# CODEJIN/multi_speaker_tts

Hardware: AMD Instinct MI355X
Metric: mel-frames/sec (train step) at batch 32x(128 tok,800 mel) (higher is better)
Workload: dtype f32

## Files before the change

include/mstts.h:

```cpp
#ifndef MSTTS_H_
#define MSTTS_H_
#include <stdint.h>
#ifdef __cplusplus
extern "C" {
#endif

typedef void* mstts_stream_t;

enum { MSTTS_OK = 0, MSTTS_ERR_SHAPE = -1, MSTTS_ERR_DTYPE = -2, MSTTS_ERR_ALIGN = -3, MSTTS_ERR_LAUNCH = -4 };
enum { MSTTS_ACT_NONE = 0, MSTTS_ACT_RELU = 1, MSTTS_ACT_TANH = 2, MSTTS_ACT_SIGMOID = 3 };

const char* mstts_last_error(void);
int mstts_abi_version(void);
int mstts_debug_park_cus(int32_t n_workgroups, int64_t microseconds, uint32_t* done_count, mstts_stream_t s);

typedef struct {
    const float* A; const float* B; float* C; const float* bias;
    int64_t M, N, K;
    int64_t lda, ldb, ldc;
    int32_t trans_a, trans_b;
    int32_t win_T, win_C, win_pad;
    int32_t act, accumulate, split_k;
    int64_t batch, stride_a, stride_b, stride_c;
    float alpha;
    int32_t win_dil;
} mstts_gemm_desc;
int mstts_gemm_f32(const mstts_gemm_desc* d, mstts_stream_t s);
int mstts_gemm_tail_split(int32_t on);
int mstts_gemm_split3(int32_t on);
int mstts_gemm_split_big(int32_t on);
int mstts_gemm_big_min_workgroups(int32_t f32_split, int32_t bf16);
int mstts_gemm_deterministic(int32_t on);
int mstts_gemm_bf16(const mstts_gemm_desc* d, mstts_stream_t s);
int mstts_gemm_bf16_autocut(int32_t on);
int mstts_gemm_bf16_big(int32_t on);

int mstts_philox_keep_mask(uint8_t* out, int64_t n, uint64_t seed, uint32_t stream_id, float keep_prob, mstts_stream_t s);
int mstts_philox_keep_mask_rows(uint8_t* out, int64_t outer, int64_t B, int64_t inner, uint64_t seed, uint32_t stream_id,
                                uint64_t sample0, float keep_prob, mstts_stream_t s);

int mstts_embedding_fwd(const int32_t* token, const float* table, float* out, int64_t n, int64_t vocab, int64_t width, mstts_stream_t s);
int mstts_embedding_bwd(const int32_t* token, const float* dout, float* dtable, int64_t n, int64_t vocab, int64_t width, mstts_stream_t s);

int mstts_bn_train_fwd(const float* x, const float* gamma, const float* beta, float* moving_mean, float* moving_var,
                       float* y, float* save_mean, float* save_rstd, const uint8_t* keep_mask, float keep_prob,
                       float momentum, float eps, int64_t rows, int64_t C, float* ws, mstts_stream_t s);
int mstts_bn_infer_fwd(const float* x, const float* gamma, const float* beta, const float* moving_mean,
                       const float* moving_var, float* y, float eps, int64_t rows, int64_t C, mstts_stream_t s);
int mstts_bn_train_bwd(const float* dy, const float* x, const float* gamma, const float* save_mean, const float* save_rstd,
                       const uint8_t* keep_mask, float keep_prob, int32_t act, float* dz, float* dgamma, float* dbeta,
                       float* dbias, int64_t rows, int64_t C, float* ws, mstts_stream_t s);

#define MSTTS_BN_SEG_MAX 16
typedef struct { const float* gamma; const float* beta; float* moving_mean; float* moving_var; } mstts_bn_seg;
typedef struct { mstts_bn_seg seg[MSTTS_BN_SEG_MAX]; } mstts_bn_seg_table;
int mstts_bn_train_fwd_seg(const float* x, int64_t ld, const mstts_bn_seg_table* segs, int32_t nseg, float* y, float* save_mean,
                           float* save_rstd, float momentum, float eps, int64_t rows, int64_t C, int64_t pool_T, float* ws, mstts_stream_t s);
#define MSTTS_BANK_MAX 16
typedef struct { const float* kernel[MSTTS_BANK_MAX]; const float* bias[MSTTS_BANK_MAX]; } mstts_convbank_src;
int mstts_convbank_pack(const mstts_convbank_src* src, int32_t bank_k, int32_t k_split, int64_t cin, int64_t cout, float* w, float* bias,
                        mstts_stream_t s);

int mstts_dropout(const float* x, const uint8_t* keep_mask, float keep_prob, float* y, int64_t n, mstts_stream_t s);
int mstts_relu_dropout_bwd(const float* dy, const float* y_saved, const uint8_t* keep_mask, float keep_prob, float* dx, int64_t n, mstts_stream_t s);
int mstts_colsum(const float* x, int64_t rows, int64_t C, int64_t ld, float* out, int32_t accumulate, mstts_stream_t s);
int mstts_add(const float* a, const float* b, float* y, int64_t n, mstts_stream_t s);
int mstts_fill(float* y, float v, int64_t n, mstts_stream_t s);
int mstts_persist_status(const uint32_t* ctrl_a, int32_t done_a, const uint32_t* ctrl_b, int32_t done_b, int32_t* flag, mstts_stream_t s);
// ... 424 lines not shown
```

multi_speaker_tts_amd/csrc/gemm.hip:

```cpp
#include "gemm_tile.h"
#include <type_traits>
#include <cmath>
#include <cstdlib>

namespace mstts {

constexpr int BK = 32;
constexpr int BN = 128;

struct GemmArgs : GemmTileArgs {
    int body, tail_s, tail_kps;
    int band;
};

template <int R, bool VEC>
struct LoaderKC {
    static constexpr int NV = R * BK / 4 / 256;
    float4 reg[NV];
    const float* ubase;
    unsigned voff[NV], rmask;
    int t_row[NV], tap, kc, ld_;
    __device__ __forceinline__ void prepare(const float* __restrict__ base, long ld, int row0, int k0, int rows,
                                            int wT, int wC, int wpad, int wdil) {
        const int k4 = threadIdx.x & 7, r = threadIdx.x >> 3;
// ... 224 lines not shown
}

template <int BM>
struct GemmF32 {
    using Args = GemmArgs;
    static constexpr int THREADS = 256;
    static constexpr size_t LDS_BYTES = 0;
    template <bool TA, bool TB, bool VEC, bool WIN> static constexpr auto kernel() { return &gemm_kernel<BM, TA, TB, VEC>; }
};

#include "gemm_split.inc"

}

using namespace mstts;

static int g_tail_split = 1;
extern "C" int mstts_gemm_tail_split(int32_t on) { g_tail_split = on != 0; return MSTTS_OK; }
static int g_split3 = 1;
extern "C" int mstts_gemm_split3(int32_t on) { g_split3 = on != 0; return MSTTS_OK; }
static int g_split_big = 1;
extern "C" int mstts_gemm_split_big(int32_t on) { g_split_big = on != 0; return MSTTS_OK; }
static int g_split_big_min = 160;
namespace mstts { void gemm_bf16_set_big_min(int n); }
extern "C" int mstts_gemm_big_min_workgroups(int32_t f32_split, int32_t bf16) {
    if (f32_split > 0) g_split_big_min = f32_split;
    gemm_bf16_set_big_min(bf16);
    return MSTTS_OK;
}
static thread_local int t_deterministic = 0;
extern "C" int mstts_gemm_deterministic(int32_t on) { t_deterministic = on != 0; return MSTTS_OK; }
namespace mstts { int gemm_deterministic_now() { return t_deterministic; } }

extern "C" int mstts_gemm_f32(const mstts_gemm_desc* d, mstts_stream_t stream) {
    GemmArgs g;
    bool vec;
    const int rc = gemm_args_from(d, "gemm", BK, 1 << 24, &g, &vec);
    if (rc != MSTTS_OK || g.M == 0 || g.N == 0) return rc;
    const int batch = d->batch > 0 ? (int)d->batch : 1, split = g.split_k, kps = g.k_per_split;
    const bool skinny = d->M <= 32;
    int bm = skinny ? 32 : 128, tail_s = 1, tail_rem = 0;
    const bool split3 = g_split3 && !skinny && d->K >= 160 && (d->win_T <= 0 || (d->win_T >= BK && d->win_C >= BK)) && gemm_ready<GemmSplit>();
    if (!skinny) {
        const double t128 = (double)cdiv(d->M, 128) * cdiv(d->N, BN) * batch * split, t64 = (double)cdiv(d->M, 64) * cdiv(d->N, BN) * batch * split;
        const double e128 = t128 / (ceil(t128 / 256.0) * 256.0), e64 = t64 / (ceil(t64 / 256.0) * 256.0);
        if (e64 * 0.95 > e128 && !split3) bm = 64;
        if (g_tail_split && !t_deterministic && batch == 1 && split == 1 && (d->act == MSTTS_ACT_NONE || !d->accumulate)) {
            double best = (bm == 128 ? ceil(t128 / 256.0) : ceil(t64 / 256.0) * 0.54);
            const int ktiles = cdiv(d->K, BK);
            for (int cand = 128; cand >= (split3 ? 128 : 64); cand -= 64) {
                const long t = (long)cdiv(d->M, cand) * cdiv(d->N, BN);
                int rem = (int)(t % 256);
                if (d->act != MSTTS_ACT_NONE) rem = (int)(t - (t - rem) / cdiv(d->N, BN) * cdiv(d->N, BN));
                if (split3 && t <= 128) rem = (int)t;
                else if (t <= 256 || rem == 0 || rem > 128) continue;
                int s = 256 / rem;
                if (s > 16) s = 16;
                if (s > ktiles / 8) s = ktiles / 8;
                if (s < 2) continue;
                const double c = ((double)(t / 256) + 1.25 / s + 0.06) * (cand == 128 ? 1.0 : 0.54);
                if (c < best) { best = c; bm = cand; tail_s = s; tail_rem = rem; }
            }
        }
    }
    hipStream_t st = (hipStream_t)stream;
    const bool ta = d->trans_a != 0, tb = d->trans_b != 0, win = g.win_T > 0;
    {
        const long big_wgs = (long)cdiv(d->M, GSB_BM) * cdiv(d->N, GSB_BN) * batch * split;
        if (split3 && g_split_big && d->M >= 192 && d->N >= 192 && big_wgs >= g_split_big_min && d->lda < (1 << 22) && d->ldb < (1 << 22) &&
            (d->win_T <= 0 || (d->win_T >= GSB_BK && d->win_C >= GSB_BK)) && (d->act == MSTTS_ACT_NONE || split == 1) && gemm_ready<GemmSplitBig>()) {
            const int kpsb = gemm_k_per_split(g.K, split, GSB_BK);
            g.k_per_split = kpsb;
            g.body = 0; g.tail_s = 1; g.tail_kps = kpsb; g.band = 0;
            dim3 gridb(cdiv(d->M, GSB_BM) * cdiv(d->N, GSB_BN), 1, batch * split);
            gemm_launch<GemmSplitBig>(g, ta, tb, vec, win, gridb, st);
            MSTTS_CHECK_LAUNCH("gemm_f32 (split, 256 x 256 tile)");
            return MSTTS_OK;
        }
    }
    const int tiles = cdiv(d->M, bm) * cdiv(d->N, BN);
    g.body = tiles; g.tail_s = 1; g.tail_kps = kps;
    g.band = (split3 && tail_s == 1 && cdiv(d->N, BN) > 8) ? 8 : 0;
    if (tail_s > 1) {
        const int rem = tail_rem, tiles_n = cdiv(d->N, BN);
        g.body = tiles - rem; g.tail_s = tail_s;
        g.tail_kps = (cdiv(g.K, BK) + tail_s - 1) / tail_s * BK;
        if (!d->accumulate) {
            const long r0 = (long)(g.body / tiles_n) * bm;
            if (hipMemset2DAsync(d->C + r0 * d->ldc, (size_t)d->ldc * 4, 0, (size_t)d->N * 4, (size_t)(d->M - r0), st) != hipSuccess)
                MSTTS_REQUIRE(false, MSTTS_ERR_LAUNCH, "gemm: clearing the tail tiles failed");
        }
    }
    dim3 grid(g.body + (tiles - g.body) * g.tail_s, 1, batch * split);
    if (split3) gemm_launch<GemmSplit>(g, ta, tb, vec, win, grid, st);
    else if (skinny) gemm_launch<GemmF32<32>>(g, ta, tb, vec, win, grid, st);
    else if (bm == 64) gemm_launch<GemmF32<64>>(g, ta, tb, vec, win, grid, st);
    else gemm_launch<GemmF32<128>>(g, ta, tb, vec, win, grid, st);
    MSTTS_CHECK_LAUNCH("gemm_f32");
    if (tail_s > 1 && d->act != MSTTS_ACT_NONE) {
        const long r0 = (long)(g.body / cdiv(d->N, BN)) * bm;
        const long n = (d->M - r0) * d->N;
        hipLaunchKernelGGL(gemm_tail_act_kernel, dim3((unsigned)cdiv(n, 256)), dim3(256), 0, st, d->C + r0 * d->ldc, d->ldc, (int)d->N, n, d->act);
        MSTTS_CHECK_LAUNCH("gemm_f32 tail activation");
    }
    return MSTTS_OK;
}
```

multi_speaker_tts_amd/csrc/gemm_split.inc:

```

typedef __bf16 gs_bf16x8 __attribute__((ext_vector_type(8)));
typedef __bf16 gs_bf16x4 __attribute__((ext_vector_type(4)));
constexpr int GS_BM = 128, GS_LD = 40;
constexpr int GS_PLANE = 128 * GS_LD;

struct Split3 { gs_bf16x4 hi, mid, lo; };
__device__ __forceinline__ uint32_t gs_cvt_pk(float a, float b) {
    uint32_t r;
    asm("v_cvt_pk_bf16_f32 %0, %1, %2" : "=v"(r) : "v"(a), "v"(b));
    return r;
}
__device__ __forceinline__ float gs_sub(float a, uint32_t b_bits) {
    float r;
    asm("v_sub_f32 %0, %1, %2" : "=v"(r) : "v"(a), "v"(b_bits));
    return r;
}
__device__ __forceinline__ void gs_split2(float x0, float x1, uint32_t& hi, uint32_t& mid, uint32_t& lo) {
    hi = gs_cvt_pk(x0, x1);
    x0 = gs_sub(x0, hi << 16); x1 = gs_sub(x1, hi & 0xffff0000u);
    mid = gs_cvt_pk(x0, x1);
    x0 = gs_sub(x0, mid << 16); x1 = gs_sub(x1, mid & 0xffff0000u);
    lo = gs_cvt_pk(x0, x1);
}
__device__ __forceinline__ Split3 gs_split4(float a, float b, float c, float d) {
// ... 123 lines not shown
    auto products = [&](int set) {
#pragma unroll
        for (int tt = 0; tt < GS_NPROD; ++tt) {
            const int pa = (tt == 0) ? 0 : (tt == 1) ? 1 : (tt == 2) ? 0 : (tt == 3) ? 1 : (tt == 4) ? 2 : 0;
            const int pb = (tt == 0) ? 0 : (tt == 1) ? 0 : (tt == 2) ? 1 : (tt == 3) ? 1 : (tt == 4) ? 0 : 2;
#pragma unroll
            for (int i = 0; i < 2; ++i)
#pragma unroll
                for (int j = 0; j < 2; ++j)
                    acc[i][j] = __builtin_amdgcn_mfma_f32_32x32x16_bf16(fa[set][i][pa], fb[set][j][pb], acc[i][j], 0, 0, 0);
        }
    };
    GS_BAR(0);
    frags(0, gs_lds, 0);
    for (int t = 0; t < nt2; ++t) {
        const __bf16* buf = gs_lds + (t & 1) * GS_BUF;
        frags(1, buf, 1);
        __builtin_amdgcn_sched_barrier(0);
        products(0);
        __builtin_amdgcn_sched_barrier(0);
        GS_BAR(0);
        frags(0, gs_lds + ((t + 1) & 1) * GS_BUF, 0);
        __builtin_amdgcn_sched_barrier(0);
        products(1);
        __builtin_amdgcn_sched_barrier(0);
    }
#ifdef GS_STAMP
    if (stamp && (threadIdx.x & 63) == 0) { unsigned long long* o = (unsigned long long*)g.bias; o[0] = acc_wait; o[1] = __builtin_readcyclecounter() - t_begin; o[2] = nt2; o[3] = wall_clock64() - w_begin; }
    if (stamp) return;
#endif
    gemm_store_tile<2, 2>(g, acc, C, m0 + wrow, n0 + wcol, lane, split == 0 && piece <= 0, g.split_k > 1 || piece >= 0);
}

constexpr int GSB_BM = 256, GSB_BN = 256, GSB_BK = 16, GSB_LD = 24, GSB_THREADS = 512;
constexpr int GSB_PLANE = 256 * GSB_LD;
constexpr int GSB_BUF = 6 * GSB_PLANE;
constexpr size_t GSB_LDS_BYTES = 2 * GSB_BUF * sizeof(__bf16);
template <bool VEC, bool WIN> using GsbLoaderKC = TileLoaderKC<4, 2, 128, GSB_LD, SplitPlanes<GSB_PLANE>, VEC, WIN>;
template <bool VEC, bool WIN> using GsbLoaderMC = TileLoaderMC<4, GSB_LD, SplitPlanes<GSB_PLANE>, VEC, WIN>;

template <bool TRANSPOSED, int HALF>
__device__ __forceinline__ bool gsb_stages(int tid) {
    if (TRANSPOSED) return (tid >> 8) == HALF;
    return true;
}

template <bool TA, bool TB, bool VEC, bool WIN>
__global__ __launch_bounds__(GSB_THREADS) void gemm_split_big_kernel(GemmArgs g) {
    extern __shared__ __attribute__((aligned(16))) __bf16 gs_lds[];
    const int tiles_n = (g.N + GSB_BN - 1) / GSB_BN;
    const int tile = gemm_xcd_tile(blockIdx.x, gridDim.x);
    const int tile_m = tile / tiles_n, tile_n = tile % tiles_n;
    const int batch = blockIdx.z / g.split_k, split = blockIdx.z % g.split_k;
    float* C = g.C + (long)batch * g.stride_c;
    const int m0 = tile_m * GSB_BM, n0 = tile_n * GSB_BN;
    const int kbeg = split * g.k_per_split;
    const int kend = min(g.K, kbeg + g.k_per_split);
    const int nt = kend > kbeg ? (kend - kbeg + GSB_BK - 1) / GSB_BK : 0;
    const int tid = threadIdx.x, lane = tid & 63, wave = __builtin_amdgcn_readfirstlane(tid >> 6);
    const int wrow = (wave >> 2) * 128, wcol = (wave & 3) * 64;
    const int l31 = lane & 31, kg = lane >> 5;

    using LA = typename std::conditional<TA, GsbLoaderMC<VEC, WIN>, GsbLoaderKC<VEC, WIN>>::type;
    using LB = typename std::conditional<TB, GsbLoaderKC<VEC, false>, GsbLoaderMC<VEC, false>>::type;
    LA la; LB lb;
    const bool a_mine = gsb_stages<TA, 0>(tid), b_mine = gsb_stages<!TB, 1>(tid);
    const int tid_a = TA ? (tid & 255) : tid, tid_b = TB ? tid : (tid & 255);
    if (a_mine) la.prepare(tid_a, g.A + (long)batch * g.stride_a, g.lda, m0, kbeg, g.M, g.win_T, g.win_C, g.win_pad, g.win_dil);
    if (b_mine) lb.prepare(tid_b, g.B + (long)batch * g.stride_b, g.ldb, n0, kbeg, g.N, 0, 1, 0, 1);
    float4 ra[4], rb[4];
    auto load = [&](int k) {
        if (a_mine) la.load(tid_a, ra, k, kend, g.lda, g.win_T, g.win_C, g.win_pad, g.win_dil);
        if (b_mine) lb.load(tid_b, rb, k, kend, g.ldb, 0, 1, 0, 1);
    };
    auto store = [&](int buf) {
        if (a_mine) la.store(tid_a, ra, gs_lds + buf * GSB_BUF);
        if (b_mine) lb.store(tid_b, rb, gs_lds + buf * GSB_BUF + 3 * GSB_PLANE);
    };

    f32x16 acc[4][2];
#pragma unroll
    for (int i = 0; i < 4; ++i)
#pragma unroll
        for (int j = 0; j < 2; ++j)
#pragma unroll
            for (int r = 0; r < 16; ++r) acc[i][j][r] = 0.f;

    const int aoff = (wrow + l31) * GSB_LD + kg * 8, boff = 3 * GSB_PLANE + (wcol + l31) * GSB_LD + kg * 8;
    gs_bf16x8 fb[2][3], fa0[4], fa1[4];
    auto ldA = [&](gs_bf16x8 (&f)[4], const __bf16* buf, int p) {
#pragma unroll
        for (int i = 0; i < 4; ++i) f[i] = *reinterpret_cast<const gs_bf16x8*>(buf + aoff + p * GSB_PLANE + i * 32 * GSB_LD);
    };
    auto ldB = [&](const __bf16* buf) {
#pragma unroll
        for (int p = 0; p < 3; ++p)
#pragma unroll
            for (int j = 0; j < 2; ++j) fb[j][p] = *reinterpret_cast<const gs_bf16x8*>(buf + boff + p * GSB_PLANE + j * 32 * GSB_LD);
    };
    auto mm = [&](const gs_bf16x8 (&f)[4], int pb) {
#pragma unroll
        for (int i = 0; i < 4; ++i)
#pragma unroll
            for (int j = 0; j < 2; ++j)
                acc[i][j] = __builtin_amdgcn_mfma_f32_32x32x16_bf16(f[i], fb[j][pb], acc[i][j], 0, 0, 0);
    };

    if (nt > 0) {
        load(kbeg);
        store(0);
        load(kbeg + GSB_BK);
        gemm_barrier();
        for (int t = 0; t < nt; ++t) {
            const __bf16* buf = gs_lds + (t & 1) * GSB_BUF;
            ldB(buf); ldA(fa0, buf, 0); ldA(fa1, buf, 1);
            mm(fa0, 0); mm(fa0, 1); mm(fa0, 2);
            ldA(fa0, buf, 2);
            store((t + 1) & 1);
            load(kbeg + (t + 2) * GSB_BK);
            mm(fa1, 0); mm(fa1, 1);
            mm(fa0, 0);
            gemm_barrier();
        }
    }
    gemm_store_tile<4, 2>(g, acc, C, m0 + wrow, n0 + wcol, lane, split == 0, g.split_k > 1);
}

struct GemmSplit {
    using Args = GemmArgs;
    static constexpr int THREADS = GS_THREADS;
    static constexpr size_t LDS_BYTES = GS_LDS_BYTES;
    template <bool TA, bool TB, bool VEC, bool WIN> static constexpr auto kernel() { return &gemm_split_kernel<TA, TB, VEC, WIN>; }
};
struct GemmSplitBig {
    using Args = GemmArgs;
    static constexpr int THREADS = GSB_THREADS;
    static constexpr size_t LDS_BYTES = GSB_LDS_BYTES;
    template <bool TA, bool TB, bool VEC, bool WIN> static constexpr auto kernel() { return &gemm_split_big_kernel<TA, TB, VEC, WIN>; }
};
```

multi_speaker_tts_amd/engine.py:

```python
from __future__ import annotations

import ctypes as C
import os
import warnings

import numpy as np
import torch

from . import lib
from .lib import ACT_NONE, ACT_RELU, ACT_TANH, gemm, ptr, call
from .masks import MaskSet, step_seed
from .params import CELL, ENC_CELL, LSA, LSA_VARS, VOC, Dims, ParamStore, bank_groups, bank_suffix
from .persist import PERSIST_COOLDOWN, PERSIST_STRIKES, CoolDown, Ticket, decoder_workgroups, lstm_bwd_workgroups, lstm_fwd_workgroups, near_xcd
from .training import (BN_EPS, BN_MOM, Engine, _split_k, _split_k_big, bn_train_fwd, conv_bn_bwd, conv_fwd, exponential_decay, lstm_layer_grads,
                       lstm_seq_bwd, lstm_seq_fwd)

MAX_PLANS = 64



def learning_rate(step):
    from . import Hyper_Parameters as hp
    return exponential_decay(hp.Train.Learning_Rate, step)


VOC_OVERLAP = os.environ.get("MSTTS_VOC_OVERLAP", "1") != "0"
VOC_FUSED = os.environ.get("MSTTS_VOC_FUSED", "1") != "0"
POSTNET_WGRAD_OVERLAP = os.environ.get("MSTTS_POSTNET_WGRAD_OVERLAP", "1") != "0"
ENC_TAIL_OVERLAP = os.environ.get("MSTTS_ENC_TAIL_OVERLAP", "1") != "0"
ENC_OVERLAP = os.environ.get("MSTTS_ENC_OVERLAP", "1") != "0"


class _WS:
    """Attribute bag of device buffers for one (B, T_enc, L) shape: views into the engine's workspace arena."""


class _LateScalars:

    def __init__(self, event, slot, wr_rate):
        self.event, self.slot, self.wr_rate, self._res = event, slot, wr_rate, None

    def get(self):
        if self._res is None:
            self.event.synchronize()
            s = self.slot.numpy().copy()
            wr = float(s[3]) * self.wr_rate
            self._res = {"Linear_Loss": float(s[0]), "Postnet_Loss": float(s[1]), "Stop_Loss": float(s[2]),
                         "Weight_Regularization_Loss": wr, "Loss": float(s[0] + s[1] + s[2]) + wr}
        return self._res


class _Arena:

    ALIGN = 256

    def __init__(self, device):
        self.device, self.buf, self.cap, self.generation = device, None, 0, 0

    def ensure(self, nbytes):
        if nbytes <= self.cap:
            return False
        self.buf = None
# ... 87 lines not shown
        self.persist_bwd_selftest = 0
        self.persist_stamps = None
        self.persist_bwd = self.persist and os.environ.get("MSTTS_PERSIST_BWD", "1") != "0" and bool(lb.mstts_persist_bwd_supported(1, H, M, d.att, 1, d.att_k))
        self.persist_bwd_fallbacks = 0
        self.ctx_dead = d.spk if d.spk == 256 and M == 2 * d.enc_lstm + d.spk else 0
        self.speaker_ticket_redos = 0
        self.trace_events, self.bptt_end_event = False, None
        self.collective_redos = 0
        self.persist_bwd_stamps = None
        if self.persist:
            self.pk = [self._f(int(lb.mstts_persist_pack_floats(i))) for i in range(3)]
        self.persist_enc = os.environ.get("MSTTS_PERSIST_ENC", "1") != "0" and bool(lb.mstts_persist_lstm_supported(1, He))
        self.persist_enc_fallbacks = 0
        if self.persist_enc:
            n = int(lb.mstts_persist_lstm_pack_floats())
            self.enc_pk = {dr: (self._f(n), self._f(n)) for dr in ("fw", "bw")}
        if self.device.type == "cuda":
            self._side = torch.cuda.Stream(device=self.device)
            self._enc_stream = torch.cuda.Stream(device=self.device)
            self._voc_stream = self._enc_stream
        if self.persist_bwd:
            self.pkb = [self._f(int(lb.mstts_persist_bwd_pack_floats(i))) for i in range(3)]
        self.flip = {}
        self.voc_bank = None
        if update_vocoder_bn and d.bank_ch % 4 == 0 and d.n_mel % 4 == 0 and 1 <= d.bank_k <= lib.BANK_MAX:
            groups = bank_groups(d.bank_k, max(1, d.bank_k // 2))
            n = sum(win * d.n_mel * (hi - lo + 1) * d.bank_ch for lo, hi, win, _ in groups)
            self.voc_bank = {"groups": groups, "w": self._f(n), "bias": self._f(d.bank_k * d.bank_ch), "version": None, "tables": None}
        self.big_tiles = os.environ.get("MSTTS_SPLIT_K_BIG", "1") != "0"
        self._derived_stale = True
        self.gemm_dtype = (gemm_dtype or "f32").lower()
        if self.gemm_dtype not in ("f32", "bf16"):
            raise ValueError("gemm_dtype must be 'f32' or 'bf16'")
        self.recurrent_dtype = (recurrent_dtype or "f32").lower()
        if self.recurrent_dtype not in ("f32", "bf16"):
            raise ValueError("recurrent_dtype must be 'f32' or 'bf16'")
        self.bf = None
        if self.recurrent_dtype == "bf16" and lb.mstts_cell_fwd_bf16_supported(H, M + H) and lb.mstts_cell_fwd_bf16_supported(H, 2 * H):
            self.w0p16 = torch.zeros((M + H) * 4 * H, dtype=torch.int16, device=self.device)
            self.w1p16 = torch.zeros(2 * H * 4 * H, dtype=torch.int16, device=self.device)
        if self.recurrent_dtype == "bf16":
            sp = (C.c_int32 * 6)()
            if not lib.load().mstts_decoder_bf16_splits(H, M, d.att, sp):
                raise ValueError("bf16 recurrent products need dec_lstm, mem and att widths that are multiples of 64")
            i16 = lambda n: torch.zeros(n, dtype=torch.int16, device=self.device)
            self.bf = {"splits": list(sp), "w0f_f": i16((M + H) * 4 * H), "w1_f": i16(2 * H * 4 * H), "wq_f": i16(H * d.att),
                       "w0f_b": i16((M + H) * 4 * H), "w1_b": i16(2 * H * 4 * H), "wq_b": i16(H * d.att)}

    def _gemm(self, *a, exact=False, **k):
        bf = self.gemm_dtype == "bf16" and not exact
        if self.deterministic and k.get("split_k", 1) > 1:
            k["split_k"], k["accumulate"] = 1, True
        if k.get("split_k", 1) > 1 and self.big_tiles:
            big = _split_k_big(a[3], a[4], a[5], None)
            if big is not None:
                k["split_k"] = max(2, big)
            elif bf:
                k["split_k"], k["accumulate"] = 1, True
        return gemm(*a, bf16=bf, **k)

    def _ensure_fallback_packs(self):
        if not getattr(self, "_fallback_packs_stale", True):
            return
        self._fallback_packs_stale = False
        d = self.d
        H, M = d.dec_lstm, d.mem
# ... 168 lines not shown
        w.mel_out = f(B, S, d.n_mel)
        w.bn_ws = f(2 * max(d.post_ch, d.enc_conv_ch, d.bank_k * d.bank_ch, d.proj1_ch, d.n_mel, d.emb))
        if self.update_vocoder_bn:
            w.voc_fused = VOC_FUSED and self.voc_bank is not None
            if not w.voc_fused:
                w.v_tmp = f(B * S, d.bank_ch)
                w.v_tmp2 = f(B * S, d.bank_ch)
                w.v_p2y = f(B * S, d.n_mel)
            w.v_cat = f(B * S, d.bank_k * d.bank_ch)
            w.v_pool = f(B * S, d.bank_k * d.bank_ch)
            w.v_p1 = f(B * S, d.proj1_ch)
            w.v_p1y = f(B * S, d.proj1_ch)
            w.v_p2 = f(B * S, d.n_mel)
            widest = max(d.bank_k * d.bank_ch if w.voc_fused else d.bank_ch, d.proj1_ch, d.n_mel)
            w.v_stat = f(2 * widest)
            w.v_bn_ws = f(4 * widest)
        w.scalars = f(4)
        w.d_linear, w.d_post, w.d_stop = f(B, S, d.n_mel), f(B, S, d.n_mel), f(B, S)
        w.post_dz = [f(B * S, c) for c in chans]
        w.post_dx = f(B * S, max(d.post_ch, d.n_mel))
        w.post_dx2 = f(B * S, max(d.post_ch, d.n_mel))
        w.d_proj = f(S, B, self.proj_ld)
        w.d_pj = f(S, B, H + M, zero=bool(self.ctx_dead))
        w.dg0, w.dg1 = f(S, B, 4 * H), f(S, B, 4 * H)
        w.dq_hist, w.de_hist = f(S, B, A), f(S, B, Te)
        w.d_in0_parts = int(lb.mstts_decoder_train_bwd_parts(H, M))
        w.d_in0 = f(w.d_in0_parts, S, B, M + H, zero=bool(self.ctx_dead))
        w.dec_bwd_ws = f(int(lb.mstts_decoder_train_bwd_ws_floats(B, H, M, A, Te, d.att_ch)), zero=True)
        w.lsa_param_ws = f((int(lb.mstts_lsa_param_bwd_ws_floats(B, Te, S)) + 3) // 4 * 4)
        w.d_pre = f(S * B, Pn)
        w.d_pre2 = f(S * B, Pn)
        w.d_keys = f(B, Te, A)
        w.d_values = f(B, Te, M, zero=bool(self.ctx_dead))
        w.enc_dgs = {dr: f(Te, B, 4 * He) for dr in ("fw", "bw")}
        w.enc_dgp = {dr: f(B, Te, 4 * He) for dr in ("fw", "bw")}
        w.enc_bwd_ws = {dr: f(int(lb.mstts_lstm_seq_ws_floats(B, He, 1))) for dr in ("fw", "bw")}
        w.enc_dy = f(B * Te, max(d.enc_conv_ch, d.emb))
        w.enc_dz = f(B * Te, d.enc_conv_ch)
        w.enc_dx = f(B * Te, max(d.enc_conv_ch, d.emb))
        w.job_flag = cv.take(1, dtype=torch.int32)
        w.job_flag_host = self._pin("job_flag_host", 1)
        w.dec = lib.DecoderTrain()
        w.dec_b = lib.DecoderTrainBwd()
        w.dec_b.ctx_dead = self.ctx_dead
        if w.persist_bwd:
            w.pdesc_b.ctx_dead = self.ctx_dead
        w.zero_on_activate = cv.zero
        w.extent_bytes = cv.off
        w.arena_generation = self._arena.generation
        return (None if (cv.count or cv.overflow) else w), cv.off

    def forward(self, batch, w, seed=None, masks=None, _redo=False, allowed=None, overlap_vocoder=False):
        d, ps = self.d, self.params
        B, Te, L, S = w.B, w.Te, w.L, w.S
        H, M, A, Pn, He = d.dec_lstm, d.mem, d.att, d.prenet, d.enc_lstm
        w.voc_done = None
        if self._active_plan is not w and not _redo:
            self._activate(w)
        if self._derived_stale:
            self.refresh_derived()
        allowed = False if _redo else (self._persist_begin_step() if allowed is None else bool(allowed))
        w.persist_now = bool(w.persist) and allowed
        w.persist_bwd_now = bool(getattr(w, "persist_bwd", False)) and allowed
        speculative = (allowed and (w.persist_now or bool(getattr(w, "persist_enc", False)))) or (not _redo and "_speaker_ticket" in batch)
        if speculative:
            n_mov = self.params.n_moving
# ... 455 lines not shown
            passed = passed and job_ok
        else:
            passed = self._pass_verdict(passed, agree, _redo)
        if not passed:
            if on_abort is not None:
                on_abort()
            torch.cuda.current_stream().synchronize()
            return self.loss_and_backward(w, grad_scale=grad_scale, on_ready=on_ready, on_abort=on_abort, agree=agree, agree_async=agree_async, _redo=True)

    def _pass_verdict(self, passed, agree, redo):
        if agree is not None and not redo:
            mine = passed
            passed = bool(agree(passed))
            if mine and not passed:
                self.collective_redos += 1
        return passed

    def _recurrent_wgrads(self, w, lo, hi, part="all"):
        d = self.d
        B, Te = w.B, w.Te
        H, M, A, Pn = d.dec_lstm, d.mem, d.att, d.prenet
        n = (hi - lo) * B
        r = lo * B
        if part in ("all", "attention"):
            gsw, ogsw = self.G(LSA + "score_layer/weight_w"); gsb, ogsb = self.G(LSA + "score_layer/bias_b")
            call("mstts_lsa_param_bwd", C.byref(w.dec.lsa), hi - lo, ptr(w.q_hist, r * A), ptr(w.cum_hist, r * Te), ptr(w.de_hist, r * Te), ptr(w.d_keys),
                 ptr(self.d_loc_k), ptr(gsw, ogsw), ptr(gsb, ogsb), ptr(w.lsa_param_ws))
        if part == "attention":
            return
        g1, og1 = self.G(CELL % 1 + "kernel"); gb1, ogb1 = self.G(CELL % 1 + "bias")
        g0, og0 = self.G(CELL % 0 + "kernel"); gb0, ogb0 = self.G(CELL % 0 + "bias")
        call("mstts_colsum", ptr(w.dg1, r * 4 * H), n, 4 * H, 4 * H, ptr(gb1, ogb1), 1)
        call("mstts_colsum", ptr(w.dg0, r * 4 * H), n, 4 * H, 4 * H, ptr(gb0, ogb0), 1)
        self._gemm(w.in0, w.dg0, self.dw0f, M + H, 4 * H, n, M + H, 4 * H, 4 * H, trans_a=True, split_k=_split_k(M + H, 4 * H, n), accumulate=True,
             a_off=r * (M + H), b_off=r * 4 * H)
        self._gemm(w.in1, w.dg1, g1, 2 * H, 4 * H, n, 2 * H, 4 * H, 4 * H, trans_a=True, split_k=_split_k(2 * H, 4 * H, n), accumulate=True,
             a_off=r * 2 * H, b_off=r * 4 * H, c_off=og1)
        self._gemm(w.pre_d[-1], w.dg0, g0, Pn, 4 * H, n, Pn, 4 * H, 4 * H, trans_a=True, split_k=max(2, _split_k(Pn, 4 * H, n)),
             a_off=r * Pn, b_off=r * 4 * H, c_off=og0)
        k0, o0 = self.P(CELL % 0 + "kernel")
        self._gemm(w.dg0, k0, w.d_pre, n, Pn, 4 * H, 4 * H, 4 * H, Pn, trans_b=True, a_off=r * 4 * H, b_off=o0, c_off=r * Pn)
        gq, ogq = self.G(LSA + "query_layer/kernel")
        self._gemm(w.pj, w.dq_hist, gq, H, A, n, H + M, A, A, trans_a=True, split_k=max(2, _split_k(H, A, n)), a_off=r * (H + M), b_off=r * A, c_off=ogq)

    def _grad_range(self, *prefixes):
        ps = self.params
        offs = [(ps.offset[n], ps.offset[n] + (int(np.prod(ps.shape[n])) + 3) // 4 * 4) for n, _, _ in ps.table
                if ps.trainable[n] and n.startswith(prefixes)]
        return min(o for o, _ in offs), max(e for _, e in offs)

    def adam_step(self, grad_scale=1.0):
        lr = learning_rate(self.global_step)
        self._adam(lr, self.wr_rate, grad_scale)
        self._derived_stale = True
        self.refresh_derived()
        return lr

    def moving_stat_ranges(self):
        ps = self.params
        r = sorted((ps.offset[n], ps.offset[n] + (int(np.prod(ps.shape[n])) + 3) // 4 * 4) for n, _, _ in ps.table
                   if not ps.trainable[n] and n.endswith(("moving_mean", "moving_variance")))
        out = []
        for lo, hi in r:
            if out and out[-1][1] == lo:
                out[-1][1] = hi
            else:
                out.append([lo, hi])
        return [tuple(x) for x in out]
# ... 70 lines not shown
```

multi_speaker_tts_amd/lib.py:

```python
from __future__ import annotations

import ctypes as C
import os

import torch

from .params import LSA_VARS

_HERE = os.path.dirname(os.path.abspath(__file__))
LIB_PATH = os.path.join(_HERE, "libmstts_hip.so")

ACT_NONE, ACT_RELU, ACT_TANH, ACT_SIGMOID = 0, 1, 2, 3

vp, i64, i32, f32, u64, u32 = C.c_void_p, C.c_int64, C.c_int32, C.c_float, C.c_uint64, C.c_uint32


class GemmDesc(C.Structure):
    _fields_ = [("A", vp), ("B", vp), ("C", vp), ("bias", vp),
                ("M", i64), ("N", i64), ("K", i64), ("lda", i64), ("ldb", i64), ("ldc", i64),
                ("trans_a", i32), ("trans_b", i32), ("win_T", i32), ("win_C", i32), ("win_pad", i32),
                ("act", i32), ("accumulate", i32), ("split_k", i32),
                ("batch", i64), ("stride_a", i64), ("stride_b", i64), ("stride_c", i64), ("alpha", f32), ("win_dil", i32)]


# ... 80 lines not shown
    _fields_ = [("fwd", C.POINTER(DecoderTrain)), ("d_pj", vp), ("dg0", vp), ("dg1", vp), ("dq_hist", vp),
                ("de_hist", vp), ("d_in0", vp), ("ws", vp), ("ctx_dead", i32)]


class DecoderInfer(C.Structure):
    _fields_ = [("B", i64), ("H", i64), ("P", i64), ("n_mel", i64), ("Smax", i64), ("lsa", LsaConst),
                ("pw0", vp), ("pb0", vp), ("pw1", vp), ("pb1", vp), ("pm0", vp), ("pm1", vp), ("prenet_keep", f32),
                ("wx0", vp), ("b0", vp), ("w0f", vp), ("w1", vp), ("b1", vp), ("wq", vp), ("wproj", vp), ("bproj", vp),
                ("zoneout", f32), ("in0", vp), ("in1", vp), ("pj", vp), ("c0", vp), ("c1", vp), ("cum", vp),
                ("pre_ws", vp), ("linear", vp), ("stop", vp), ("align_hist", vp), ("w0s", vp), ("wp_pad", vp), ("w0sp", vp), ("w1p", vp), ("act_p", vp), ("wp_own", vp), ("vp", vp)]


BN_SEG_MAX = BANK_MAX = 16


class BnSeg(C.Structure):
    _fields_ = [("gamma", vp), ("beta", vp), ("moving_mean", vp), ("moving_var", vp)]


class BnSegTable(C.Structure):
    _fields_ = [("seg", BnSeg * BN_SEG_MAX)]


class ConvBankSrc(C.Structure):
    _fields_ = [("kernel", vp * BANK_MAX), ("bias", vp * BANK_MAX)]


P = C.POINTER
SIGNATURES = {
    "mstts_last_error": (C.c_char_p, []),
    "mstts_abi_version": (i32, []),
    "mstts_debug_park_cus": (i32, [i32, i64, vp, vp]),
    "mstts_gemm_f32": (i32, [P(GemmDesc), vp]),
    "mstts_gemm_tail_split": (i32, [i32]),
    "mstts_gemm_split3": (i32, [i32]),
    "mstts_gemm_deterministic": (i32, [i32]),
    "mstts_gemm_split_big": (i32, [i32]),
    "mstts_gemm_big_min_workgroups": (i32, [i32, i32]),
    "mstts_gemm_bf16_autocut": (i32, [i32]),
    "mstts_persist_status": (i32, [vp, i32, vp, i32, vp, vp]),
    "mstts_gemm_bf16": (i32, [P(GemmDesc), vp]),
    "mstts_gemm_bf16_big": (i32, [i32]),
    "mstts_philox_keep_mask": (i32, [vp, i64, u64, u32, f32, vp]),
    "mstts_philox_keep_mask_rows": (i32, [vp, i64, i64, i64, u64, u32, u64, f32, vp]),
    "mstts_embedding_fwd": (i32, [vp, vp, vp, i64, i64, i64, vp]),
    "mstts_embedding_bwd": (i32, [vp, vp, vp, i64, i64, i64, vp]),
    "mstts_bn_train_fwd": (i32, [vp, vp, vp, vp, vp, vp, vp, vp, vp, f32, f32, f32, i64, i64, vp, vp]),
    "mstts_bn_train_fwd_seg": (i32, [vp, i64, P(BnSegTable), i32, vp, vp, vp, f32, f32, i64, i64, i64, vp, vp]),
    "mstts_convbank_pack": (i32, [P(ConvBankSrc), i32, i32, i64, i64, vp, vp, vp]),
    "mstts_bn_infer_fwd": (i32, [vp, vp, vp, vp, vp, vp, f32, i64, i64, vp]),
    "mstts_bn_train_bwd": (i32, [vp, vp, vp, vp, vp, vp, f32, i32, vp, vp, vp, vp, i64, i64, vp, vp]),
    "mstts_dropout": (i32, [vp, vp, f32, vp, i64, vp]),
    "mstts_relu_dropout_bwd": (i32, [vp, vp, vp, f32, vp, i64, vp]),
    "mstts_colsum": (i32, [vp, i64, i64, i64, vp, i32, vp]),
    "mstts_add": (i32, [vp, vp, vp, i64, vp]),
    "mstts_fill": (i32, [vp, f32, i64, vp]),
    "mstts_copy2d": (i32, [vp, i64, vp, i64, i64, i64, i32, vp]),
    "mstts_maxpool2_same": (i32, [vp, vp, i64, i64, i64, vp]),
    "mstts_highway_combine": (i32, [vp, vp, vp, vp, i64, vp]),
    "mstts_maxpool2_same_bwd": (i32, [vp, vp, vp, i64, i64, i64, vp]),
    "mstts_highway_combine_bwd": (i32, [vp, vp, vp, vp, vp, vp, vp, i64, vp]),
    "mstts_l1_loss_fwd_bwd": (i32, [vp, vp, i64, vp, vp, vp]),
    "mstts_lstm_point_fwd": (i32, [P(LstmPointFwd), vp]),
    "mstts_lstm_point_bwd": (i32, [P(LstmPointBwd), vp]),
    "mstts_cell_fwd_supported": (i32, [i64, i64]),
    "mstts_pack_cell_fwd": (i32, [vp, i64, vp, i64, i64, vp]),
# ... 274 lines not shown
```

Baseline: 666,900.

## Factor attention-context weight gradient through alignments instead of materialized context rows

The context rows of the decoder LSTM input are alignment-weighted sums of encoder values. Their weight gradient is now computed as values^T · (align^T · dgates) rather than as a GEMM over every step's context vector. A per-batch intermediate Z (Te x 4H) is formed first with a new 128x256 split-bf16 tile variant, then reduced against the values with a tuned split-k. The path is enabled only when a cost heuristic predicts fewer flops, and it adds a workspace buffer and a different summation order.

```diff
diff --git a/include/mstts.h b/include/mstts.h
--- a/include/mstts.h
+++ b/include/mstts.h
@@ -34,6 +34,10 @@
 int mstts_gemm_bf16(const mstts_gemm_desc* d, mstts_stream_t s);
 int mstts_gemm_bf16_autocut(int32_t on);
 int mstts_gemm_bf16_big(int32_t on);
+int mstts_ctx_wgrad_f32(const float* align, const float* values, const float* dgates, float* Z, float* out, int64_t ldo,
+                        int64_t S, int64_t B, int64_t Te, int64_t M, int64_t N, int64_t lo, int64_t hi, mstts_stream_t s);
+int32_t mstts_ctx_wgrad_prefers_factored(int64_t B, int64_t Te, int64_t steps, int64_t M);
+int mstts_ctx_wgrad_wide_tile(int32_t on);
 
 int mstts_philox_keep_mask(uint8_t* out, int64_t n, uint64_t seed, uint32_t stream_id, float keep_prob, mstts_stream_t s);
 int mstts_philox_keep_mask_rows(uint8_t* out, int64_t outer, int64_t B, int64_t inner, uint64_t seed, uint32_t stream_id,
diff --git a/multi_speaker_tts_amd/csrc/gemm.hip b/multi_speaker_tts_amd/csrc/gemm.hip
--- a/multi_speaker_tts_amd/csrc/gemm.hip
+++ b/multi_speaker_tts_amd/csrc/gemm.hip
@@ -280,7 +280,10 @@
 extern "C" int mstts_gemm_deterministic(int32_t on) { t_deterministic = on != 0; return MSTTS_OK; }
 namespace mstts { int gemm_deterministic_now() { return t_deterministic; } }
 
-extern "C" int mstts_gemm_f32(const mstts_gemm_desc* d, mstts_stream_t stream) {
+static int g_ctx_wide = 1;
+extern "C" int mstts_ctx_wgrad_wide_tile(int32_t on) { g_ctx_wide = on != 0; return MSTTS_OK; }
+
+static int gemm_f32_run(const mstts_gemm_desc* d, mstts_stream_t stream, bool wide) {
     GemmArgs g;
     bool vec;
     const int rc = gemm_args_from(d, "gemm", BK, 1 << 24, &g, &vec);
@@ -313,6 +316,16 @@
     }
     hipStream_t st = (hipStream_t)stream;
     const bool ta = d->trans_a != 0, tb = d->trans_b != 0, win = g.win_T > 0;
+    if (wide && split3 && d->lda < (1 << 22) && d->ldb < (1 << 22) && (d->win_T <= 0 || (d->win_T >= GSB_BK && d->win_C >= GSB_BK)) &&
+        (d->act == MSTTS_ACT_NONE || split == 1) && gemm_ready<GemmSplitWide>()) {
+        const int kpsw = gemm_k_per_split(g.K, split, GSB_BK);
+        g.k_per_split = kpsw;
+        g.body = 0; g.tail_s = 1; g.tail_kps = kpsw; g.band = 0;
+        dim3 gridw(cdiv(d->M, GSW_BM) * cdiv(d->N, GSB_BN), 1, batch * split);
+        gemm_launch<GemmSplitWide>(g, ta, tb, vec, win, gridw, st);
+        MSTTS_CHECK_LAUNCH("gemm_f32 (split, 128 x 256 tile)");
+        return MSTTS_OK;
+    }
     {
         const long big_wgs = (long)cdiv(d->M, GSB_BM) * cdiv(d->N, GSB_BN) * batch * split;
         if (split3 && g_split_big && d->M >= 192 && d->N >= 192 && big_wgs >= g_split_big_min && d->lda < (1 << 22) && d->ldb < (1 << 22) &&
@@ -353,3 +366,62 @@
     }
     return MSTTS_OK;
 }
+
+extern "C" int mstts_gemm_f32(const mstts_gemm_desc* d, mstts_stream_t stream) { return gemm_f32_run(d, stream, false); }
+
+static const double CTX_WGRAD_MARGIN = 2.0;
+extern "C" int32_t mstts_ctx_wgrad_prefers_factored(int64_t B, int64_t Te, int64_t steps, int64_t M) {
+    if (B <= 0 || Te <= 0 || steps <= 1 || M <= 0) return 0;
+    const double rows = (double)steps * (double)B;
+    return CTX_WGRAD_MARGIN * ((double)Te * rows + (double)M * (double)B * (double)Te) <= (double)M * rows;
+}
+
+static int ctx_wgrad_cut(long M, long N, long K) {
+    if (g_split3 && g_split_big && M >= 192 && N >= 192 && K >= 160) {
+        const long tiles = (long)cdiv(M, GSB_BM) * cdiv(N, GSB_BN);
+        int best = 0;
+        double best_cost = 0.0;
+        for (int sk = 1; sk <= 64; ++sk) {
+            if (sk > 1 && K / sk < 1024) break;
+            if (tiles * sk < g_split_big_min) continue;
+            const double cost = (double)cdiv(tiles * sk, 256L) * ((double)K / sk + 300.0) * (1.0 + 0.01 * sk);
+            if (best == 0 || cost < best_cost - 1e-9) { best = sk; best_cost = cost; }
+        }
+        if (best > 0) return best;
+    }
+    const long tiles = (long)cdiv(M, 128) * cdiv(N, BN);
+    int best = 1;
+    double best_cost = 0.0;
+    for (int sk = 1; sk <= 16; ++sk) {
+        if (sk > 1 && K / sk < 512) break;
+        const double cost = (double)cdiv(tiles * sk, 256L) / sk + 0.004 * sk;
+        if (sk == 1 || cost < best_cost - 1e-9) { best = sk; best_cost = cost; }
+    }
+    return best;
+}
+
+extern "C" int mstts_ctx_wgrad_f32(const float* align, const float* values, const float* dgates, float* Z, float* out, int64_t ldo,
+                                   int64_t S, int64_t B, int64_t Te, int64_t M, int64_t N, int64_t lo, int64_t hi, mstts_stream_t stream) {
+    MSTTS_REQUIRE(S >= 0 && B >= 0 && Te >= 0 && M >= 0 && N >= 0, MSTTS_ERR_SHAPE, "ctx_wgrad: negative dims");
+    MSTTS_REQUIRE(lo >= 0 && hi <= S, MSTTS_ERR_SHAPE, "ctx_wgrad: step range [%lld, %lld) outside [0, %lld)", (long long)lo, (long long)hi, (long long)S);
+    const int64_t s0 = lo > 1 ? lo : 1;
+    if (hi <= s0 || B == 0 || Te == 0 || M == 0 || N == 0) return MSTTS_OK;
+    MSTTS_REQUIRE(align && values && dgates && Z && out, MSTTS_ERR_SHAPE, "ctx_wgrad: null operand");
+    MSTTS_REQUIRE(ldo >= N, MSTTS_ERR_SHAPE, "ctx_wgrad: output row pitch below its width");
+    MSTTS_REQUIRE(B < 65536 && B * Te < (1LL << 31), MSTTS_ERR_SHAPE, "ctx_wgrad: batch of 65 536 or more, or B . Te beyond int32");
+    mstts_gemm_desc d = {};
+    d.A = align + (s0 - 1) * B * Te; d.B = dgates + s0 * B * N; d.C = Z;
+    d.M = Te; d.N = N; d.K = hi - s0;
+    d.lda = B * Te; d.ldb = B * N; d.ldc = N;
+    d.trans_a = 1; d.split_k = 1; d.alpha = 1.f;
+    d.batch = B; d.stride_a = Te; d.stride_b = N; d.stride_c = Te * N;
+    const int rc = gemm_f32_run(&d, stream, g_ctx_wide != 0);
+    if (rc != MSTTS_OK) return rc;
+    d = mstts_gemm_desc{};
+    d.A = values; d.B = Z; d.C = out;
+    d.M = M; d.N = N; d.K = B * Te;
+    d.lda = M; d.ldb = N; d.ldc = ldo;
+    d.trans_a = 1; d.accumulate = 1; d.alpha = 1.f;
+    d.split_k = t_deterministic ? 1 : ctx_wgrad_cut(M, N, B * Te);
+    return mstts_gemm_f32(&d, stream);
+}
diff --git a/multi_speaker_tts_amd/csrc/gemm_split.inc b/multi_speaker_tts_amd/csrc/gemm_split.inc
--- a/multi_speaker_tts_amd/csrc/gemm_split.inc
+++ b/multi_speaker_tts_amd/csrc/gemm_split.inc
@@ -179,39 +179,41 @@
     gemm_store_tile<2, 2>(g, acc, C, m0 + wrow, n0 + wcol, lane, split == 0 && piece <= 0, g.split_k > 1 || piece >= 0);
 }
 
-constexpr int GSB_BM = 256, GSB_BN = 256, GSB_BK = 16, GSB_LD = 24, GSB_THREADS = 512;
-constexpr int GSB_PLANE = 256 * GSB_LD;
-constexpr int GSB_BUF = 6 * GSB_PLANE;
-constexpr size_t GSB_LDS_BYTES = 2 * GSB_BUF * sizeof(__bf16);
-template <bool VEC, bool WIN> using GsbLoaderKC = TileLoaderKC<4, 2, 128, GSB_LD, SplitPlanes<GSB_PLANE>, VEC, WIN>;
-template <bool VEC, bool WIN> using GsbLoaderMC = TileLoaderMC<4, GSB_LD, SplitPlanes<GSB_PLANE>, VEC, WIN>;
-
-template <bool TRANSPOSED, int HALF>
+constexpr int GSB_BM = 256, GSW_BM = 128, GSB_BN = 256, GSB_BK = 16, GSB_LD = 24, GSB_THREADS = 512;
+constexpr int gsb_plane(int rows) { return rows * GSB_LD; }
+constexpr int gsb_buf(int bm) { return 3 * (gsb_plane(bm) + gsb_plane(GSB_BN)); }
+constexpr size_t GSB_LDS_BYTES = 2 * gsb_buf(GSB_BM) * sizeof(__bf16), GSW_LDS_BYTES = 2 * gsb_buf(GSW_BM) * sizeof(__bf16);
+template <int ROWS, bool VEC, bool WIN> using GsbLoaderKC = TileLoaderKC<4, ROWS / 128, 128, GSB_LD, SplitPlanes<gsb_plane(ROWS)>, VEC, WIN>;
+template <int ROWS, bool VEC, bool WIN> using GsbLoaderMC = TileLoaderMC<4, GSB_LD, SplitPlanes<gsb_plane(ROWS)>, VEC, WIN>;
+
+template <bool TRANSPOSED, int HALF, int ROWS>
 __device__ __forceinline__ bool gsb_stages(int tid) {
-    if (TRANSPOSED) return (tid >> 8) == HALF;
+    if (TRANSPOSED) return ROWS == 256 ? (tid >> 8) == HALF : (tid >> 7) == 2 * HALF;
     return true;
 }
 
-template <bool TA, bool TB, bool VEC, bool WIN>
+template <int BM, bool TA, bool TB, bool VEC, bool WIN>
 __global__ __launch_bounds__(GSB_THREADS) void gemm_split_big_kernel(GemmArgs g) {
+    constexpr int WM = BM / 64;
+    constexpr int A_PLANE = gsb_plane(BM), B_PLANE = gsb_plane(GSB_BN), GSB_BUF = gsb_buf(BM);
     extern __shared__ __attribute__((aligned(16))) __bf16 gs_lds[];
     const int tiles_n = (g.N + GSB_BN - 1) / GSB_BN;
     const int tile = gemm_xcd_tile(blockIdx.x, gridDim.x);
     const int tile_m = tile / tiles_n, tile_n = tile % tiles_n;
     const int batch = blockIdx.z / g.split_k, split = blockIdx.z % g.split_k;
     float* C = g.C + (long)batch * g.stride_c;
-    const int m0 = tile_m * GSB_BM, n0 = tile_n * GSB_BN;
+    const int m0 = tile_m * BM, n0 = tile_n * GSB_BN;
     const int kbeg = split * g.k_per_split;
     const int kend = min(g.K, kbeg + g.k_per_split);
     const int nt = kend > kbeg ? (kend - kbeg + GSB_BK - 1) / GSB_BK : 0;
     const int tid = threadIdx.x, lane = tid & 63, wave = __builtin_amdgcn_readfirstlane(tid >> 6);
-    const int wrow = (wave >> 2) * 128, wcol = (wave & 3) * 64;
+    const int wrow = (wave >> 2) * (BM / 2), wcol = (wave & 3) * 64;
     const int l31 = lane & 31, kg = lane >> 5;
 
-    using LA = typename std::conditional<TA, GsbLoaderMC<VEC, WIN>, GsbLoaderKC<VEC, WIN>>::type;
-    using LB = typename std::conditional<TB, GsbLoaderKC<VEC, false>, GsbLoaderMC<VEC, false>>::type;
+    using LA = typename std::conditional<TA, GsbLoaderMC<BM, VEC, WIN>, GsbLoaderKC<BM, VEC, WIN>>::type;
+    using LB = typename std::conditional<TB, GsbLoaderKC<GSB_BN, VEC, false>, GsbLoaderMC<GSB_BN, VEC, false>>::type;
     LA la; LB lb;
-    const bool a_mine = gsb_stages<TA, 0>(tid), b_mine = gsb_stages<!TB, 1>(tid);
+    const bool a_mine = gsb_stages<TA, 0, BM>(tid), b_mine = gsb_stages<!TB, 1, GSB_BN>(tid);
     const int tid_a = TA ? (tid & 255) : tid, tid_b = TB ? tid : (tid & 255);
     if (a_mine) la.prepare(tid_a, g.A + (long)batch * g.stride_a, g.lda, m0, kbeg, g.M, g.win_T, g.win_C, g.win_pad, g.win_dil);
     if (b_mine) lb.prepare(tid_b, g.B + (long)batch * g.stride_b, g.ldb, n0, kbeg, g.N, 0, 1, 0, 1);
@@ -222,32 +224,32 @@
     };
     auto store = [&](int buf) {
         if (a_mine) la.store(tid_a, ra, gs_lds + buf * GSB_BUF);
-        if (b_mine) lb.store(tid_b, rb, gs_lds + buf * GSB_BUF + 3 * GSB_PLANE);
-    };
-
-    f32x16 acc[4][2];
-#pragma unroll
-    for (int i = 0; i < 4; ++i)
+        if (b_mine) lb.store(tid_b, rb, gs_lds + buf * GSB_BUF + 3 * A_PLANE);
+    };
+
+    f32x16 acc[WM][2];
+#pragma unroll
+    for (int i = 0; i < WM; ++i)
 #pragma unroll
         for (int j = 0; j < 2; ++j)
 #pragma unroll
             for (int r = 0; r < 16; ++r) acc[i][j][r] = 0.f;
 
-    const int aoff = (wrow + l31) * GSB_LD + kg * 8, boff = 3 * GSB_PLANE + (wcol + l31) * GSB_LD + kg * 8;
-    gs_bf16x8 fb[2][3], fa0[4], fa1[4];
-    auto ldA = [&](gs_bf16x8 (&f)[4], const __bf16* buf, int p) {
-#pragma unroll
-        for (int i = 0; i < 4; ++i) f[i] = *reinterpret_cast<const gs_bf16x8*>(buf + aoff + p * GSB_PLANE + i * 32 * GSB_LD);
+    const int aoff = (wrow + l31) * GSB_LD + kg * 8, boff = 3 * A_PLANE + (wcol + l31) * GSB_LD + kg * 8;
+    gs_bf16x8 fb[2][3], fa0[WM], fa1[WM];
+    auto ldA = [&](gs_bf16x8 (&f)[WM], const __bf16* buf, int p) {
+#pragma unroll
+        for (int i = 0; i < WM; ++i) f[i] = *reinterpret_cast<const gs_bf16x8*>(buf + aoff + p * A_PLANE + i * 32 * GSB_LD);
     };
     auto ldB = [&](const __bf16* buf) {
 #pragma unroll
         for (int p = 0; p < 3; ++p)
 #pragma unroll
-            for (int j = 0; j < 2; ++j) fb[j][p] = *reinterpret_cast<const gs_bf16x8*>(buf + boff + p * GSB_PLANE + j * 32 * GSB_LD);
-    };
-    auto mm = [&](const gs_bf16x8 (&f)[4], int pb) {
-#pragma unroll
-        for (int i = 0; i < 4; ++i)
+            for (int j = 0; j < 2; ++j) fb[j][p] = *reinterpret_cast<const gs_bf16x8*>(buf + boff + p * B_PLANE + j * 32 * GSB_LD);
+    };
+    auto mm = [&](const gs_bf16x8 (&f)[WM], int pb) {
+#pragma unroll
+        for (int i = 0; i < WM; ++i)
 #pragma unroll
             for (int j = 0; j < 2; ++j)
                 acc[i][j] = __builtin_amdgcn_mfma_f32_32x32x16_bf16(f[i], fb[j][pb], acc[i][j], 0, 0, 0);
@@ -270,7 +272,7 @@
             gemm_barrier();
         }
     }
-    gemm_store_tile<4, 2>(g, acc, C, m0 + wrow, n0 + wcol, lane, split == 0, g.split_k > 1);
+    gemm_store_tile<WM, 2>(g, acc, C, m0 + wrow, n0 + wcol, lane, split == 0, g.split_k > 1);
 }
 
 struct GemmSplit {
@@ -283,5 +285,11 @@
     using Args = GemmArgs;
     static constexpr int THREADS = GSB_THREADS;
     static constexpr size_t LDS_BYTES = GSB_LDS_BYTES;
-    template <bool TA, bool TB, bool VEC, bool WIN> static constexpr auto kernel() { return &gemm_split_big_kernel<TA, TB, VEC, WIN>; }
-};
+    template <bool TA, bool TB, bool VEC, bool WIN> static constexpr auto kernel() { return &gemm_split_big_kernel<GSB_BM, TA, TB, VEC, WIN>; }
+};
+struct GemmSplitWide {
+    using Args = GemmArgs;
+    static constexpr int THREADS = GSB_THREADS;
+    static constexpr size_t LDS_BYTES = GSW_LDS_BYTES;
+    template <bool TA, bool TB, bool VEC, bool WIN> static constexpr auto kernel() { return &gemm_split_big_kernel<GSW_BM, TA, TB, VEC, WIN>; }
+};
diff --git a/multi_speaker_tts_amd/engine.py b/multi_speaker_tts_amd/engine.py
--- a/multi_speaker_tts_amd/engine.py
+++ b/multi_speaker_tts_amd/engine.py
@@ -28,6 +28,7 @@
 VOC_FUSED = os.environ.get("MSTTS_VOC_FUSED", "1") != "0"
 POSTNET_WGRAD_OVERLAP = os.environ.get("MSTTS_POSTNET_WGRAD_OVERLAP", "1") != "0"
 ENC_TAIL_OVERLAP = os.environ.get("MSTTS_ENC_TAIL_OVERLAP", "1") != "0"
+CTX_WGRAD_ORDER = os.environ.get("MSTTS_CTX_WGRAD_ORDER", "first")
 ENC_OVERLAP = os.environ.get("MSTTS_ENC_OVERLAP", "1") != "0"
 
 
@@ -181,6 +182,7 @@
         self.gemm_dtype = (gemm_dtype or "f32").lower()
         if self.gemm_dtype not in ("f32", "bf16"):
             raise ValueError("gemm_dtype must be 'f32' or 'bf16'")
+        self.ctx_wgrad_factored = True
         self.recurrent_dtype = (recurrent_dtype or "f32").lower()
         if self.recurrent_dtype not in ("f32", "bf16"):
             raise ValueError("recurrent_dtype must be 'f32' or 'bf16'")
@@ -415,6 +417,8 @@
         w.d_pre2 = f(S * B, Pn)
         w.d_keys = f(B, Te, A)
         w.d_values = f(B, Te, M, zero=bool(self.ctx_dead))
+        w.ctx_wgrad = self.gemm_dtype == "f32" and bool(lb.mstts_ctx_wgrad_prefers_factored(B, Te, S, M))
+        w.ctx_z = f(B, Te, 4 * H) if w.ctx_wgrad else None
         w.enc_dgs = {dr: f(Te, B, 4 * He) for dr in ("fw", "bw")}
         w.enc_dgp = {dr: f(B, Te, 4 * He) for dr in ("fw", "bw")}
         w.enc_bwd_ws = {dr: f(int(lb.mstts_lstm_seq_ws_floats(B, He, 1))) for dr in ("fw", "bw")}
@@ -936,8 +940,18 @@
         g0, og0 = self.G(CELL % 0 + "kernel"); gb0, ogb0 = self.G(CELL % 0 + "bias")
         call("mstts_colsum", ptr(w.dg1, r * 4 * H), n, 4 * H, 4 * H, ptr(gb1, ogb1), 1)
         call("mstts_colsum", ptr(w.dg0, r * 4 * H), n, 4 * H, 4 * H, ptr(gb0, ogb0), 1)
-        self._gemm(w.in0, w.dg0, self.dw0f, M + H, 4 * H, n, M + H, 4 * H, 4 * H, trans_a=True, split_k=_split_k(M + H, 4 * H, n), accumulate=True,
-             a_off=r * (M + H), b_off=r * 4 * H)
+        factored = self.ctx_wgrad_factored and getattr(w, "ctx_wgrad", False) and self.gemm_dtype == "f32"
+        m0 = M if factored else 0
+
+        def context_rows():
+            call("mstts_ctx_wgrad_f32", ptr(w.align_hist), ptr(w.values), ptr(w.dg0), ptr(w.ctx_z), ptr(self.dw0f), 4 * H,
+                 w.align_hist.shape[0], B, Te, M, 4 * H, lo, hi)
+        if factored and CTX_WGRAD_ORDER == "first":
+            context_rows()
+        self._gemm(w.in0, w.dg0, self.dw0f, M + H - m0, 4 * H, n, M + H, 4 * H, 4 * H, trans_a=True, split_k=_split_k(M + H - m0, 4 * H, n),
+             accumulate=True, a_off=r * (M + H) + m0, b_off=r * 4 * H, c_off=m0 * 4 * H)
+        if factored and CTX_WGRAD_ORDER != "first":
+            context_rows()
         self._gemm(w.in1, w.dg1, g1, 2 * H, 4 * H, n, 2 * H, 4 * H, 4 * H, trans_a=True, split_k=_split_k(2 * H, 4 * H, n), accumulate=True,
              a_off=r * 2 * H, b_off=r * 4 * H, c_off=og1)
         self._gemm(w.pre_d[-1], w.dg0, g0, Pn, 4 * H, n, Pn, 4 * H, 4 * H, trans_a=True, split_k=max(2, _split_k(Pn, 4 * H, n)),
diff --git a/multi_speaker_tts_amd/lib.py b/multi_speaker_tts_amd/lib.py
--- a/multi_speaker_tts_amd/lib.py
+++ b/multi_speaker_tts_amd/lib.py
@@ -136,6 +136,9 @@
     "mstts_abi_version": (i32, []),
     "mstts_debug_park_cus": (i32, [i32, i64, vp, vp]),
     "mstts_gemm_f32": (i32, [P(GemmDesc), vp]),
+    "mstts_ctx_wgrad_f32": (i32, [vp, vp, vp, vp, vp, i64, i64, i64, i64, i64, i64, i64, i64, vp]),
+    "mstts_ctx_wgrad_prefers_factored": (i32, [i64, i64, i64, i64]),
+    "mstts_ctx_wgrad_wide_tile": (i32, [i32]),
     "mstts_gemm_tail_split": (i32, [i32]),
     "mstts_gemm_split3": (i32, [i32]),
     "mstts_gemm_deterministic": (i32, [i32]),
```

Result: no change. 671,700, median of 6 (+0.7%).
